# openclimatefix/predict_pv_yield

Measured on AMD Instinct MI355X. Metric: PV-site samples/sec (train step), conv3d 12->6 frames, higher is better.
Workload: dtype bf16; 1 GPU; conv3d train step (fwd + NMAE + bwd + Adam): sat [B,11,18,64,64] N(0,1), 4x Conv3d(3x3x3, 32ch) + fc 128/128/64, 128.6 M params; per_gpu_batch=32, global_batch=32, t_frames=18, parallelism=single

## Files before the change

predict_pv_yield_amd/csrc/linear_bf16.hip:

```cpp
#include "adam.h"
#include <string.h>

namespace pv {

template <int MT>
__global__ __launch_bounds__(256) void linear_fwd_bf16_kernel(const uint16_t* __restrict__ x,
                                                               const uint16_t* __restrict__ w,
                                                               float* __restrict__ partial, int m, int n,
                                                               long long k, int kblocks_per_wg) {
  const int lane = threadIdx.x & 63;
  const int wave = threadIdx.x >> 6;
  const int r = lane & 31, hh = lane >> 5;
  const int nt = blockIdx.y * 4 + wave;
  const long long total_kb = (k + 63) / 64;
  const long long kb0 = (long long)blockIdx.x * kblocks_per_wg;
  long long kb1 = kb0 + kblocks_per_wg;
  if (kb1 > total_kb) kb1 = total_kb;

  int wrow = nt * 32 + r;
  if (wrow > n - 1) wrow = n - 1;
  const uint16_t* wp = w + (size_t)wrow * k + 32 * hh;
  const uint16_t* xp[MT];
#pragma unroll
  for (int mt = 0; mt < MT; ++mt) {
// ... 450 lines not shown
#pragma unroll
    for (int q = 0; q < 4; ++q) {
      const uint16_t h0 = f32_to_bf16_bits(gx[2 * q]), h1 = f32_to_bf16_bits(gx[2 * q + 1]);
      const uint16_t l0 = f32_to_bf16_bits(gx[2 * q] - bf16_bits_to_f32(h0)), l1 = f32_to_bf16_bits(gx[2 * q + 1] - bf16_bits_to_f32(h1));
      hw[q] = (uint32_t)h0 | ((uint32_t)h1 << 16);
      lw[q] = (uint32_t)l0 | ((uint32_t)l1 << 16);
    }
    const bf16x8 bw = *reinterpret_cast<const bf16x8*>(wt + (32 * wave + col) * FD_WLD + 16 * st + 8 * half);
    o = __builtin_amdgcn_mfma_f32_32x32x16_bf16(__builtin_bit_cast(bf16x8, lw), bw, o, 0, 0, 0);
    o = __builtin_amdgcn_mfma_f32_32x32x16_bf16(__builtin_bit_cast(bf16x8, hw), bw, o, 0, 0, 0);
  }
  __syncthreads();
#pragma unroll
  for (int r = 0; r < 16; ++r) {
    const int b = (r & 3) + 8 * (r >> 2) + 4 * half;
    xs[b * FD_XLD + 32 * wave + col] = f32_to_bf16_bits(o[r]);
  }
  __syncthreads();
  for (int i = tid; i < 32 * (FD_KT / 8); i += 256) {
    const int b = i / (FD_KT / 8), c = i - b * (FD_KT / 8);
    if (b < m && k0 + 8 * c < k) {
      u32x4 o = *reinterpret_cast<const u32x4*>(xs + b * FD_XLD + 8 * c);
      if (gate_dx) {
        const u32x4 xv = *reinterpret_cast<const u32x4*>(x + (size_t)b * k + k0 + 8 * c);
#pragma unroll
        for (int q = 0; q < 4; ++q)
          o[q] &= __builtin_bit_cast(uint32_t, __builtin_bit_cast(u16x2_t, relu_pair01(xv[q])) * (u16x2_t){0xffff, 0xffff});
      }
      *reinterpret_cast<u32x4*>(dx + (size_t)b * k + k0 + 8 * c) = o;
    }
  }
}

constexpr int TL_XS = 320;
constexpr int TL_TS = 64 + 4;
constexpr int TL_GA = 2 * 4 * 3 * 64, TL_GD = 2 * 8 * 64;
typedef __attribute__((address_space(3))) s16x4 tl_lds_s16x4_t;
static_assert(32 * TL_XS <= FD_KT * FD_WLD * 2 && 4 * 32 * TL_TS * 4 <= FD_KT * FD_WLD * 2, "x block / transpose patches live in the weight tile's bytes");

__global__ __launch_bounds__(256) void tall_split_g_kernel(const float* __restrict__ dy, int m, int n, u32x4* __restrict__ ga,
                                                            u32x4* __restrict__ gd, int nblk) {
  const int total = nblk * (TL_GA + TL_GD);
  for (int f = blockIdx.x * blockDim.x + threadIdx.x; f < total; f += gridDim.x * blockDim.x) {
    const int mb = f / (TL_GA + TL_GD), i = f - mb * (TL_GA + TL_GD);
    float v[8];
    int term;
    if (i < TL_GA) {
      const int lane = i & 63, q = i >> 6, ks = q / 12, wave = (q / 3) & 3, r = lane & 31, hh = lane >> 5;
      term = q % 3;
#pragma unroll
      for (int j = 0; j < 8; ++j) {
        const int b = 32 * mb + 16 * ks + 8 * hh + j, nn = 32 * wave + r;
        v[j] = (b < m && nn < n) ? dy[(size_t)b * n + nn] : 0.f;
      }
    } else {
      const int i2 = i - TL_GA, lane = i2 & 63, q = i2 >> 6, st = q & 7, col = lane & 31, half = lane >> 5;
      term = q >> 3;
      const int b = 32 * mb + col;
#pragma unroll
      for (int j = 0; j < 8; ++j) {
        const int nn = 16 * st + 8 * half + j;
        v[j] = (b < m && nn < n) ? dy[(size_t)b * n + nn] : 0.f;
      }
    }
    u32x4 o;
#pragma unroll
// ... 565 lines not shown
    if (wave * 32 < n) {
#pragma unroll
      for (int ks = 0; ks < V3_KC / 16; ++ks) {
        const bf16x8 b = *reinterpret_cast<const bf16x8*>(tile + b_row + pos[ks]);
#pragma unroll
        for (int q = 0; q < MB; ++q) {
          const bf16x8 a = *reinterpret_cast<const bf16x8*>(tile + a_row + q * (32 * 256) + pos[ks]);
          acc[q] = __builtin_amdgcn_mfma_f32_32x32x16_bf16(a, b, acc[q], 0, 0, 0);
        }
      }
    }
  }
  const int col = wave * 32 + r;
  if (col < n) {
    float* dst = partial + (size_t)blockIdx.x * m * n + col;
#pragma unroll
    for (int q = 0; q < MB; ++q)
#pragma unroll
      for (int j = 0; j < 16; ++j) {
        const int row = 32 * q + (j & 3) + 8 * (j >> 2) + 4 * hh;
        if (row < m) dst[(size_t)row * n] = acc[q][j];
      }
  }
}

static int v3_split(long long k, int* tiles_per_wg, int* n_tiles) {
  const long long nt = (k + V3_KC - 1) / V3_KC;
  long long nwg = nt < 256 ? nt : 256;
  const long long per = (nt + nwg - 1) / nwg;
  nwg = (nt + per - 1) / per;
  *tiles_per_wg = (int)per;
  *n_tiles = (int)nt;
  return (int)nwg;
}

static bool v2_shapes(int m, int n) { return m <= 32 && n <= 128 && n % 16 == 0 && n >= 32; }
static int v2_split(long long k, int* tiles_per_wg, int* n_tiles) {
  const long long nt = (k + V2_KC - 1) / V2_KC;
  long long nwg = nt < 512 ? nt : 512;
  const long long per = (nt + nwg - 1) / nwg;
  nwg = (nt + per - 1) / per;
  *tiles_per_wg = (int)per;
  *n_tiles = (int)nt;
  return (int)nwg;
}

static int bf16_fwd_split(long long k, int* kblocks_per_wg) {
  long long total_kb = (k + 63) / 64;
  long long nwg = total_kb < 1024 ? total_kb : 1024;
  long long per = (total_kb + nwg - 1) / nwg;
  nwg = (total_kb + per - 1) / per;
  *kblocks_per_wg = (int)per;
  return (int)nwg;
}

}

using namespace pv;

extern "C" {

int pv_linear_bf16_workspace_bytes(int32_t m, int32_t n, int64_t k, size_t* bytes) {
  PV_REQUIRE(bytes && m > 0 && n > 0 && k > 0, PV_EINVAL, "pv_linear_bf16_workspace_bytes: bad arguments");
  int per;
  int nwg = bf16_fwd_split(k, &per);
  const size_t rows = (size_t)((m + 127) / 128) * 128;
// ... 112 lines not shown
  PV_REQUIRE(step >= 1, PV_EINVAL, "pv_linear_wgrad_adam_bf16: step must be >= 1");
  size_t lds = (size_t)m * BT * sizeof(float);
  PV_REQUIRE(lds <= 64 * 1024, PV_ESIZE, "pv_linear_wgrad_adam_bf16: m=%d too large", m);
  const AdamScalars ad = adam_scalars(lr, beta1, beta2, eps, step);
  unsigned kb = (unsigned)((k / 8 + 255) / 256);
  hipLaunchKernelGGL(linear_bwd_dw_bf16_kernel<1>, dim3(xcd_grid(kb, (unsigned)((n + BT - 1) / BT))), dim3(256), lds,
                     as_stream(stream), x, dy, y_relu_mask, param, m, n, (long long)k, exp_avg, exp_avg_sq, bf16_shadow, ad);
  return check_launch("pv_linear_wgrad_adam_bf16");
}

int pv_linear_wgrad_adam_f32(const float* x, const float* dy, const float* y_relu_mask, float* param, float* exp_avg,
                             float* exp_avg_sq, int32_t m, int32_t n, int64_t k, double lr, double beta1, double beta2,
                             double eps, int32_t step, void* stream) {
  PV_REQUIRE(x && dy && param && exp_avg && exp_avg_sq, PV_EINVAL, "pv_linear_wgrad_adam_f32: null pointer");
  PV_REQUIRE(m > 0 && n > 0 && k > 0 && k % 8 == 0, PV_ESIZE, "pv_linear_wgrad_adam_f32: bad sizes (k must be a multiple of 8)");
  PV_REQUIRE(((uintptr_t)x % 16) == 0 && ((uintptr_t)param % 16) == 0 && ((uintptr_t)exp_avg % 16) == 0 && ((uintptr_t)exp_avg_sq % 16) == 0,
             PV_EINVAL, "pv_linear_wgrad_adam_f32: 16-byte aligned buffers expected");
  PV_REQUIRE(step >= 1, PV_EINVAL, "pv_linear_wgrad_adam_f32: step must be >= 1");
  size_t lds = (size_t)m * BT * sizeof(float);
  PV_REQUIRE(lds <= 64 * 1024, PV_ESIZE, "pv_linear_wgrad_adam_f32: m=%d too large", m);
  const AdamScalars ad = adam_scalars(lr, beta1, beta2, eps, step);
  unsigned kb = (unsigned)((k / 8 + 255) / 256);
  hipLaunchKernelGGL((linear_bwd_dw_bf16_kernel<1, float>), dim3(xcd_grid(kb, (unsigned)((n + BT - 1) / BT))), dim3(256), lds,
                     as_stream(stream), x, dy, y_relu_mask, param, m, n, (long long)k, exp_avg, exp_avg_sq, (uint16_t*)nullptr, ad);
  return check_launch("pv_linear_wgrad_adam_f32");
}

#define PV_LAUNCH_FC1_ONE_PASS(grid, st, ...)                                                                         \
  do {                                                                                                                \
    const char* fs_ = getenv("PV_FC1_FETCH");                                                                         \
    if (fs_ && !strcmp(fs_, "late")) hipLaunchKernelGGL((linear_bwd_dw_dx_adam_kernel<1, false>), dim3(grid), dim3(256), 0, st, __VA_ARGS__); \
    else if (fs_ && !strcmp(fs_, "early1")) hipLaunchKernelGGL((linear_bwd_dw_dx_adam_kernel<1, true>), dim3(grid), dim3(256), 0, st, __VA_ARGS__); \
    else if (fs_ && !strcmp(fs_, "early2")) hipLaunchKernelGGL((linear_bwd_dw_dx_adam_kernel<2, true>), dim3(grid), dim3(256), 0, st, __VA_ARGS__); \
    else hipLaunchKernelGGL((linear_bwd_dw_dx_adam_kernel<2, true, 4>), dim3(grid), dim3(256), 0, st, __VA_ARGS__);    \
  } while (0)

int pv_linear_wgrad_dx_adam_bf16(const uint16_t* x, const float* dy, const float* y_relu_mask, float* param, float* exp_avg,
                                 float* exp_avg_sq, uint16_t* bf16_shadow, uint16_t* dx, float* db, int32_t m, int32_t n,
                                 int64_t k, double lr, double beta1, double beta2, double eps, int32_t step,
                                 int32_t gate_dx_by_x, int32_t moments_tiled, void* stream) {
  PV_REQUIRE(x && dy && param && exp_avg && exp_avg_sq, PV_EINVAL, "pv_linear_wgrad_dx_adam_bf16: null pointer");
  PV_REQUIRE(m > 0 && m <= 32 && n > 0 && n <= 128 && n % 8 == 0, PV_ESIZE,
             "pv_linear_wgrad_dx_adam_bf16: built for m <= 32 rows of x and n <= 128 (multiple of 8) outputs, got m=%d n=%d", m, n);
  PV_REQUIRE(k > 0 && k % 8 == 0, PV_ESIZE, "pv_linear_wgrad_dx_adam_bf16: k must be a multiple of 8");
  PV_REQUIRE(step >= 1, PV_EINVAL, "pv_linear_wgrad_dx_adam_bf16: step must be >= 1");
  PV_REQUIRE(!moments_tiled || k % FD_KT == 0, PV_ESIZE, "pv_linear_wgrad_dx_adam_bf16: tiled moments need k %% %d == 0", FD_KT);
  const AdamScalars ad = adam_scalars(lr, beta1, beta2, eps, step);
  const unsigned grid = (unsigned)((k + FD_KT - 1) / FD_KT);
  PV_LAUNCH_FC1_ONE_PASS(grid, as_stream(stream), x, dy, y_relu_mask, param, m, n,
                     (long long)k, exp_avg, exp_avg_sq, bf16_shadow, dx, db, ad, gate_dx_by_x, (const float*)nullptr,
                     moments_tiled ? 1 : 0);
  return check_launch("pv_linear_wgrad_dx_adam_bf16");
}

int pv_linear_wgrad_dx_adam_tall_bf16_workspace_bytes(int32_t m, size_t* bytes) {
  PV_REQUIRE(m > 0 && bytes, PV_EINVAL, "pv_linear_wgrad_dx_adam_tall_bf16_workspace_bytes: bad arguments");
  *bytes = (size_t)((m + 31) / 32) * (TL_GA + TL_GD) * 16;
  return PV_OK;
}

int pv_linear_wgrad_dx_adam_tall_bf16(const uint16_t* x, const float* dy, float* param, float* exp_avg, float* exp_avg_sq,
                                      uint16_t* bf16_shadow, uint16_t* dx, int32_t m, int32_t n, int64_t k, double lr,
                                      double beta1, double beta2, double eps, int32_t step, float grad_scale,
                                      int32_t gate_dx_by_x, int32_t moments_tiled, void* workspace, size_t workspace_bytes,
                                      void* stream) {
  PV_REQUIRE(x && dy && param && exp_avg && exp_avg_sq && workspace, PV_EINVAL, "pv_linear_wgrad_dx_adam_tall_bf16: null pointer");
  PV_REQUIRE(!moments_tiled || k % FD_KT == 0, PV_ESIZE, "pv_linear_wgrad_dx_adam_tall_bf16: tiled moments need k %% 128 == 0");
// ... 59 lines not shown
```

predict_pv_yield_amd/csrc/conv3d_wgrad_bf16_v2.hip:

```cpp
#include "pv_common.h"

namespace pv {

constexpr int W2TR = 8, W2TRI = 10, W2TW = 32, W2XW = 34;
constexpr int W2_SLAB_ELEMS = 28 * 32 * 32;
constexpr uint32_t W2_INVALID = 0x40000000u;

typedef __attribute__((address_space(3))) s16x4 w2_lds_s16x4;
typedef __attribute__((address_space(3))) unsigned char* w2_lds_ptr;
typedef int w2_i32x4 __attribute__((ext_vector_type(4)));

__device__ __forceinline__ void w2_lds_dma16(uint32_t lds_addr, uint32_t voff, w2_i32x4 rsrc, uint32_t soff) {
  asm volatile("s_mov_b32 m0, %0\n\ts_nop 0\n\tbuffer_load_dwordx4 %1, %2, %3 offen lds" ::"s"(lds_addr), "v"(voff), "s"(rsrc),
               "s"(soff)
               : "memory");
}
__device__ __forceinline__ w2_i32x4 w2_rsrc(const void* base, int bytes) {
  const uintptr_t a = (uintptr_t)base;
  return (w2_i32x4){(int)(uint32_t)a, (int)((a >> 32) & 0xffffu), bytes, 0x00020000};
}

#ifdef PV_DIAG_STAMPS
__device__ unsigned long long wgrad2_diag[PV_DIAG_WAVES * PV_DIAG_SLOTS];
#endif

template <int NACC, int Q>
__device__ __forceinline__ void w2_interleave() {
  if constexpr (Q < NACC) {
    constexpr int R = 2 + 2 * NACC;
    __builtin_amdgcn_sched_group_barrier(0x008, 1, 0);
    __builtin_amdgcn_sched_group_barrier(0x100, R / NACC + (Q < R % NACC ? 1 : 0), 0);
    w2_interleave<NACC, Q + 1>();
  }
}

template <int CPAD, bool F16 = false, bool PACK12 = false>
__global__ __launch_bounds__(512, 2) void conv3d_wgrad_bf16_v2_kernel(
    const uint16_t* __restrict__ x, const uint16_t* __restrict__ dy, float* __restrict__ slabs, int t_in, int h_in, int w_in,
    int t_out, int h_out, int w_out, int pad_t, int pad_h, int pad_w, int n_colblk, int t_chunk, int rpb) {
  constexpr int NCH = CPAD / 8;
  constexpr int VPR = 16 / NCH;
  constexpr int VOXB = CPAD * 2;
  constexpr int ROWB = W2XW * VOXB;
  constexpr int SLOTB = W2TRI * ROWB;
  constexpr int XVPP = 1024 / VOXB;
  constexpr int XPIECES = (W2XW + XVPP - 1) / XVPP;
  constexpr int XTAIL_LANES = (W2XW - (XPIECES - 1) * XVPP) * NCH;
  constexpr int DROWB = W2TW * 64;
  constexpr int DSLOTB = W2TR * DROWB;
  constexpr int NXS = 5;
  __shared__ __attribute__((aligned(1024))) unsigned char lds[NXS * SLOTB + 256 + 2 * DSLOTB];
  unsigned char* lds_const = lds + NXS * SLOTB;
  unsigned char* lds_dy = lds_const + 256;

  const int tid = threadIdx.x;
  const int lane = tid & 63;
  const int wave8 = __builtin_amdgcn_readfirstlane(tid >> 6);
  const bool loader = wave8 >= 4;
  const int wave = wave8 & 3;
  const int grp = lane >> 4;
  const int qi = (lane & 15) >> 2;
  const int pi = lane & 3;
  const int hh = grp >> 1;
  const int cb = 16 * (grp & 1);

  const int h0 = blockIdx.x * rpb;
  const int b = blockIdx.z;
  const int tc0 = blockIdx.y * t_chunk;
  const int tc1 = min(tc0 + t_chunk, t_out);
  const int wg_id = (blockIdx.z * gridDim.y + blockIdx.y) * gridDim.x + blockIdx.x;
  float* slab = slabs + (size_t)wg_id * W2_SLAB_ELEMS;

  static_assert(!PACK12 || CPAD == 16, "PACK12 packs the 16-channel image");
  constexpr bool PAIRED = CPAD == 16;
  constexpr int NACC = PACK12 ? 3 : (PAIRED ? 4 : 7);
  f32x16 acc[NACC];
#pragma unroll
  for (int i = 0; i < NACC; ++i)
#pragma unroll
    for (int j = 0; j < 16; ++j) acc[i][j] = 0.f;

  const int nt = tc1 - tc0, tn = nt + 2;
  const int n_items = nt > 0 ? nt * n_colblk : 0;
  const int u_end = tn * n_colblk;
  const uint32_t lds_base = __builtin_amdgcn_readfirstlane((uint32_t)(uintptr_t)(w2_lds_ptr)lds);

  if (n_items > 0 && loader) {
    const uint32_t x_plane_b = (uint32_t)h_in * w_in * CPAD * 2u, x_row_b = (uint32_t)w_in * CPAD * 2u;
    const uint32_t d_plane_b = (uint32_t)h_out * w_out * 64u, d_row_b = (uint32_t)w_out * 64u;
    const size_t x_sample = (size_t)t_in * h_in * w_in * CPAD, d_sample = (size_t)t_out * h_out * w_out * 32;
    const void* const x_base = x + (size_t)b * x_sample;
    const void* const d_base = dy + (size_t)b * d_sample;
    const int x_bytes = (int)(x_sample * 2), d_bytes = (int)(d_sample * 2);
    uint32_t xrow_src[3];
    bool xrow_in[3];
#pragma unroll
    for (int i = 0; i < 3; ++i) {
      const int hi = h0 - pad_h + wave + 4 * i;
      xrow_in[i] = (unsigned)hi < (unsigned)h_in && wave + 4 * i < rpb + 2;
      xrow_src[i] = xrow_in[i] ? (uint32_t)hi * x_row_b : 0u;
    }
    uint32_t drow_src[2];
    bool drow_in[2];
#pragma unroll
    for (int i = 0; i < 2; ++i) {
      const int ho = h0 + wave + 4 * i;
// ... 45 lines not shown
    for (int j = 0; j < n_items; ++j) {
      const int cb = j / nt, u0 = cb * tn + (j - cb * nt);
      __builtin_amdgcn_s_waitcnt(0x0f70);
      __syncthreads();
      if (next_u < u0 + 3) {
        for (; next_u < u0 + 3; ++next_u) x_slice(next_u);
        __builtin_amdgcn_s_waitcnt(0x0f70);
        __syncthreads();
      }
      for (; next_u <= u0 + 4 && next_u < u_end; ++next_u) x_slice(next_u);
      if (j + 1 < n_items) d_slice(j + 1);
    }
  } else if (n_items > 0) {
    if (tid < 64) reinterpret_cast<uint32_t*>(lds_const)[tid] = tid < 32 ? (F16 ? 0x3c003c00u : 0x3f803f80u) : 0u;

    int aoff[2];
#pragma unroll
    for (int s = 0; s < 2; ++s) {
      const int v = 8 * hh + 4 * s + qi;
      const int chunk = (cb + 4 * pi) >> 3;
      aoff[s] = v * 64 + ((chunk ^ ((v >> 2) & 3)) << 4) + (pi & 1) * 8;
    }
    int boff[NACC][2];
    int bkt[NACC];
    int my_tap[NACC];
#pragma unroll
    for (int i = 0; i < NACC; ++i) {
      int tap, c4 = 0;
      if constexpr (PACK12) {
        const int piece = 8 * (wave + 4 * i) + 4 * (grp & 1) + pi;
        tap = piece / 3;
        c4 = piece - 3 * tap;
        if (piece > 81) tap = 28;
      } else {
        tap = PAIRED ? 2 * (wave + 4 * i) + (grp & 1) : wave + 4 * i;
      }
      my_tap[i] = tap;
      if (tap > 26) tap = 26;
      const int kt = tap / 9, kh = (tap / 3) % 3, kw = tap % 3;
      bkt[i] = kt;
      const int cbx = PAIRED ? 0 : cb;
#pragma unroll
      for (int s = 0; s < 2; ++s) {
        const int v = kw + 8 * hh + 4 * s + qi;
        const int chunk = PACK12 ? (c4 >> 1) : ((cbx + 4 * pi) >> 3);
        const int sub = PACK12 ? (c4 & 1) : (pi & 1);
        boff[i][s] = kh * ROWB + v * VOXB + ((chunk ^ ((v / VPR) % NCH)) << 4) + sub * 8;
      }
    }
    typedef __attribute__((ext_vector_type(8))) short s16x8;
    const int last_tap = (PAIRED || PACK12) ? my_tap[NACC - 1] : (wave == 3 ? 27 : 0);
    const unsigned char* const_frag = last_tap < 27 ? nullptr : lds_const + (last_tap == 27 ? 0 : 128) + (lane & 15) * 8;

#ifdef PV_DIAG_STAMPS
    unsigned long long dg[PV_DIAG_SLOTS] = {0, 0, 0, 0, 0, 0, 0, 0}, s0, s1, s2;
#endif
    for (int j = 0; j < n_items; ++j) {
      const int cbj = j / nt, u0 = cbj * tn + (j - cbj * nt);
      PV_STAMP(s0);
      __syncthreads();
      if (cbj > 0 && j == cbj * nt) __syncthreads();
      PV_STAMP(s1);
      int slot_of_kt[3];
#pragma unroll
      for (int kt = 0; kt < 3; ++kt) slot_of_kt[kt] = ((u0 + kt) % NXS) * SLOTB;
      const unsigned char* dy_slot = lds_dy + (j & 1) * DSLOTB;
      int bslot[NACC];
#pragma unroll
      for (int i = 0; i < NACC; ++i) bslot[i] = bkt[i] == 0 ? slot_of_kt[0] : (bkt[i] == 1 ? slot_of_kt[1] : slot_of_kt[2]);
      auto read_step = [&](int st, s16x4 (&ra)[2], s16x4 (&rb)[NACC][2]) {
        const int rho = st >> 1, cg = st & 1;
        const unsigned char* ap = dy_slot + rho * DROWB + cg * 16 * 64;
        ra[0] = __builtin_amdgcn_ds_read_tr16_b64_v4i16((w2_lds_s16x4*)(ap + aoff[0]));
        ra[1] = __builtin_amdgcn_ds_read_tr16_b64_v4i16((w2_lds_s16x4*)(ap + aoff[1]));
        const int xo = rho * ROWB + cg * 16 * VOXB;
#pragma unroll
        for (int i = 0; i < NACC; ++i) {
          const unsigned char* bp = lds + bslot[i] + xo;
          const unsigned char* p0 = bp + boff[i][0];
          const unsigned char* p1 = bp + boff[i][1];
          if (i == NACC - 1) {
            p0 = const_frag ? const_frag : p0;
            p1 = const_frag ? const_frag : p1;
          }
          rb[i][0] = __builtin_amdgcn_ds_read_tr16_b64_v4i16((w2_lds_s16x4*)p0);
          rb[i][1] = __builtin_amdgcn_ds_read_tr16_b64_v4i16((w2_lds_s16x4*)p1);
        }
      };
      auto mfma_step = [&](const s16x4 (&ra)[2], const s16x4 (&rb)[NACC][2]) {
        const s16x8 a8 = {ra[0][0], ra[0][1], ra[0][2], ra[0][3], ra[1][0], ra[1][1], ra[1][2], ra[1][3]};
        typedef _Float16 w2_f16x8 __attribute__((ext_vector_type(8)));
#pragma unroll
        for (int i = 0; i < NACC; ++i) {
          s16x8 t8 = {rb[i][0][0], rb[i][0][1], rb[i][0][2], rb[i][0][3], rb[i][1][0], rb[i][1][1], rb[i][1][2], rb[i][1][3]};
          if constexpr (F16)
            acc[i] = __builtin_amdgcn_mfma_f32_32x32x16_f16(__builtin_bit_cast(w2_f16x8, a8), __builtin_bit_cast(w2_f16x8, t8), acc[i], 0, 0, 0);
          else
            acc[i] = __builtin_amdgcn_mfma_f32_32x32x16_bf16(__builtin_bit_cast(bf16x8, a8), __builtin_bit_cast(bf16x8, t8), acc[i], 0, 0, 0);
        }
      };
      s16x4 ra0[2], ra1[2], rb0[NACC][2], rb1[NACC][2];
      const bool skip_last_row = rpb < W2TR;
      read_step(0, ra0, rb0);
#pragma unroll
      for (int st = 0; st < W2TR * 2; st += 2) {
        if (st == W2TR * 2 - 2 && skip_last_row) break;
        __builtin_amdgcn_sched_barrier(0);
        read_step(st + 1, ra1, rb1);
        mfma_step(ra0, rb0);
        w2_interleave<NACC, 0>();
        __builtin_amdgcn_sched_barrier(0);
        if (st + 2 < W2TR * 2) {
          read_step(st + 2, ra0, rb0);
          mfma_step(ra1, rb1);
          w2_interleave<NACC, 0>();
        } else {
          mfma_step(ra1, rb1);
        }
        __builtin_amdgcn_sched_barrier(0);
      }
#ifdef PV_DIAG_STAMPS
      PV_STAMP(s2);
      dg[0] += s1 - s0;
      dg[1] += s2 - s1;
      dg[2] += 1;
#endif
    }
#ifdef PV_DIAG_STAMPS
    if (lane == 0 && wg_id * 4 + wave < PV_DIAG_WAVES)
      for (int i = 0; i < PV_DIAG_SLOTS; ++i) wgrad2_diag[(size_t)(wg_id * 4 + wave) * PV_DIAG_SLOTS + i] = dg[i];
#endif
  }
  if (loader) return;

  const int half = lane >> 5;
#pragma unroll
  for (int i = 0; i < NACC; ++i) {
    int tapslot = PAIRED ? 2 * (wave + 4 * i) + ((lane & 31) >> 4) : wave + 4 * i;
    int ci = PAIRED ? (lane & 15) : (lane & 31);
    if constexpr (PACK12) {
      const int piece = 8 * (wave + 4 * i) + ((lane & 31) >> 2);
      tapslot = piece / 3;
      ci = 4 * (piece - 3 * tapslot) + (lane & 3);
      if (piece > 81) tapslot = 28;
    }
    if (tapslot <= 27) {
      float* dst = slab + (size_t)tapslot * 1024 + ci;
#pragma unroll
      for (int j = 0; j < 16; ++j) {
        const int co = (j & 3) + 8 * (j >> 2) + 4 * half;
        dst[co * 32] = acc[i][j];
      }
    }
  }
}

void wgrad_v2_grid(const pv_conv3d_dims* d, int* n_rowblk, int* n_colblk, int* n_tchunk, int* t_chunk, int* rows_per_blk) {
  const int to = d->t_in + 2 * d->pad_t - 2, ho = d->h_in + 2 * d->pad_h - 2, wo = d->w_in + 2 * d->pad_w - 2;
  *n_rowblk = (ho + W2TR - 1) / W2TR;
  if ((long long)d->batch * *n_rowblk < 256 && (long long)d->batch * (*n_rowblk + 1) <= 256 &&
      (ho + *n_rowblk) / (*n_rowblk + 1) < (ho + *n_rowblk - 1) / *n_rowblk)
    *n_rowblk += 1;
  *rows_per_blk = (ho + *n_rowblk - 1) / *n_rowblk;
  *n_colblk = (wo + W2TW - 1) / W2TW;
  const long long tiles = (long long)d->batch * *n_rowblk;
  int max_chunks = (to + 1) / 2;
  if (max_chunks < 1) max_chunks = 1;
  int ntc = 1;
  long long best = -1;
  for (int c = 1; c <= max_chunks && tiles * c <= 16 * 256; ++c) {
    const int tch = (to + c - 1) / c, nch = (to + tch - 1) / tch;
    const long long rounds = (tiles * nch + 255) / 256;
    const long long cost = rounds * (tch + 2);
    if (best < 0 || cost < best) best = cost, ntc = nch;
  }
  *t_chunk = (to + ntc - 1) / ntc;
  *n_tchunk = (to + *t_chunk - 1) / *t_chunk;
}

size_t wgrad_v2_workspace_bytes(const pv_conv3d_dims* d) {
  int nrb, ncb, ntc, tch, rpb;
  wgrad_v2_grid(d, &nrb, &ncb, &ntc, &tch, &rpb);
  return (size_t)d->batch * nrb * ntc * W2_SLAB_ELEMS * sizeof(float);
}

int launch_conv3d_wgrad_bf16_v2(const uint16_t* x, const uint16_t* dy, float* slabs, const pv_conv3d_dims* d, int to, int ho,
                                int wo, hipStream_t st, int* n_slabs, bool f16) {
  if (((uintptr_t)x % 16) != 0 || ((uintptr_t)dy % 16) != 0) return 1;
  int nrb, ncb, ntc, tch, rpb;
  wgrad_v2_grid(d, &nrb, &ncb, &ntc, &tch, &rpb);
  *n_slabs = d->batch * nrb * ntc;
  dim3 grid((unsigned)nrb, (unsigned)ntc, (unsigned)d->batch);
#define PV_W2(CP, HALF)                                                                                                       \
  hipLaunchKernelGGL((conv3d_wgrad_bf16_v2_kernel<CP, HALF>), grid, dim3(512), 0, st, x, dy, slabs, d->t_in, d->h_in, d->w_in, to, \
                     ho, wo, d->pad_t, d->pad_h, d->pad_w, ncb, tch, rpb)
#define PV_W2P(HALF)                                                                                                        \
  hipLaunchKernelGGL((conv3d_wgrad_bf16_v2_kernel<16, HALF, true>), grid, dim3(512), 0, st, x, dy, slabs, d->t_in, d->h_in, d->w_in, \
                     to, ho, wo, d->pad_t, d->pad_h, d->pad_w, ncb, tch, rpb)
  if (pv_bf16_cpad(d->c_in) == 16) {
    const bool pack12 = d->c_in <= 12 && !getenv("PV_WGRAD_NO_PACK12");
    if (pack12) { if (f16) PV_W2P(true); else PV_W2P(false); }
    else { if (f16) PV_W2(16, true); else PV_W2(16, false); }
  } else { if (f16) PV_W2(32, true); else PV_W2(32, false); }
#undef PV_W2P
#undef PV_W2
  return 0;
}


constexpr int WR_GROUPS = 16;
__global__ __launch_bounds__(64 * WR_GROUPS) void conv3d_wgrad_reduce_kernel(const float* __restrict__ slabs, int n_slabs,
                                                                              float* __restrict__ dw, float* __restrict__ dbias,
                                                                              int c_out, int c_in) {
  __shared__ float part[WR_GROUPS][64];
  const int lane = threadIdx.x & 63, grp = threadIdx.x >> 6;
  const int i = blockIdx.x * 64 + lane;
  float s0 = 0.f, s1 = 0.f, s2 = 0.f, s3 = 0.f;
  for (int k = grp; k < n_slabs; k += 16 * WR_GROUPS) {
    float v[16];
#pragma unroll
    for (int j = 0; j < 16; ++j) v[j] = (k + WR_GROUPS * j < n_slabs) ? slabs[(size_t)(k + WR_GROUPS * j) * W2_SLAB_ELEMS + i] : 0.f;
#pragma unroll
    for (int j = 0; j < 16; j += 4) s0 += v[j], s1 += v[j + 1], s2 += v[j + 2], s3 += v[j + 3];
  }
  part[grp][lane] = (s0 + s1) + (s2 + s3);
  __syncthreads();
  if (grp == 0) {
    float t[WR_GROUPS];
#pragma unroll
    for (int q = 0; q < WR_GROUPS; ++q) t[q] = part[q][lane];
#pragma unroll
    for (int w = WR_GROUPS / 2; w >= 1; w >>= 1)
#pragma unroll
      for (int q = 0; q < w; ++q) t[q] = t[2 * q] + t[2 * q + 1];
    const float s = t[0];
    const int tap = i >> 10, co = (i >> 5) & 31, ci = i & 31;
// ... 103 lines not shown
```

Baseline: 20650 samples/s.

## Add warp-specialized persistent FC1 backward+Adam kernel with LDS DMA ring

Adds a new specialization of the fused fc1 weight-gradient, dx and Adam kernel. It dedicates four loader waves to streaming param, exp_avg, exp_avg_sq and x tiles into a four-stage LDS ring via buffer_load...lds DMA, while eight compute waves form gradients, apply Adam and compute dx. The grid is capped at the CU count so blocks are persistent and loop over tiles. The aim is to hide the memory latency of the bandwidth-bound optimizer update for the large fc1 weight. In exchange it relies on inline asm, a barrier hand-off between loader and compute waves that must stay matched, 32-bit buffer offsets, and an environment variable fallback to the old kernel.

```diff
diff --git a/predict_pv_yield_amd/csrc/linear_bf16.hip b/predict_pv_yield_amd/csrc/linear_bf16.hip
--- a/predict_pv_yield_amd/csrc/linear_bf16.hip
+++ b/predict_pv_yield_amd/csrc/linear_bf16.hip
@@ -506,6 +506,265 @@
   }
 }
 
+constexpr int FS_CHUNKB = 3 * 16 * 512;
+constexpr int FS_LW = 4;
+constexpr int FS_CL = 24 / FS_LW;
+constexpr int FS_XL = 8 / FS_LW;
+constexpr uint32_t FS_INVALID = 0xfffffff0u;
+typedef int fs_i32x4 __attribute__((ext_vector_type(4)));
+
+__device__ __forceinline__ void fs_lds_dma16(uint32_t lds_addr, uint32_t voff, fs_i32x4 rsrc) {
+  asm volatile("s_mov_b32 m0, %0\n\ts_nop 0\n\tbuffer_load_dwordx4 %1, %2, 0 offen lds" ::"s"(lds_addr), "v"(voff), "s"(rsrc)
+               : "memory");
+}
+__device__ __forceinline__ fs_i32x4 fs_rsrc(const void* base, uint32_t bytes) {
+  const uintptr_t a = (uintptr_t)base;
+  return (fs_i32x4){(int)(uint32_t)a, (int)((a >> 32) & 0xffffu), (int)bytes, 0x00020000};
+}
+
+template <int AHEAD, bool EARLY, int GR, int STAGES, int CW>
+__global__ __launch_bounds__(64 * (CW + FS_LW), 1) void linear_bwd_dw_dx_adam_kernel(
+    const uint16_t* __restrict__ x, const float* __restrict__ dy, const float* __restrict__ ymask, float* __restrict__ w,
+    int m, int n, long long k, float* __restrict__ exp_avg, float* __restrict__ exp_avg_sq, uint16_t* __restrict__ shadow,
+    uint16_t* __restrict__ dx, float* __restrict__ db, AdamScalars ad, int gate_dx, const float* __restrict__ ad_dev,
+    int mv_tiled) {
+  static_assert(GR == 4 && STAGES == 4 && (CW == 4 || CW == 8), "the ring's hand-over below is written for four stages and gradient halves");
+  constexpr int CPT = 32 / CW;
+  constexpr int KQN = FD_KT / CPT;
+  constexpr int NT = 64 * CW;
+  __shared__ __attribute__((aligned(1024))) unsigned char ring[STAGES * FS_CHUNKB];
+  __shared__ __attribute__((aligned(16))) float gs[32 * 128];
+  __shared__ __attribute__((aligned(16))) uint16_t wt[FD_KT * FD_WLD];
+  __shared__ __attribute__((aligned(1024))) uint16_t xt[32 * FD_KT];
+  typedef __attribute__((address_space(3))) unsigned char* fs_lds_ptr;
+  const int tid = threadIdx.x, lane = tid & 63;
+  const int wave = __builtin_amdgcn_readfirstlane(tid >> 6);
+  const int n_tiles = (int)(k / FD_KT);
+  const int n_my = (n_tiles - (int)blockIdx.x + (int)gridDim.x - 1) / (int)gridDim.x;
+  const int n_steps = 8 * n_my;
+
+  if (wave >= CW) {
+    const int lw = wave - CW;
+    const uint32_t ring_base = __builtin_amdgcn_readfirstlane((uint32_t)(uintptr_t)(fs_lds_ptr)ring);
+    const uint32_t xt_base = __builtin_amdgcn_readfirstlane((uint32_t)(uintptr_t)(fs_lds_ptr)xt);
+    const uint32_t w_bytes = (uint32_t)((size_t)n * k * 4);
+    const fs_i32x4 prs = fs_rsrc(w, w_bytes), mrs = fs_rsrc(exp_avg, w_bytes), vrs = fs_rsrc(exp_avg_sq, w_bytes);
+    const fs_i32x4 xrs = fs_rsrc(x, (uint32_t)((size_t)m * k * 2));
+    const int slot = lane >> 5, pos = lane & 31;
+    const uint32_t piece_b = (uint32_t)(CW == 4 ? 2 * (pos & 15) + (pos >> 4) : pos) * 16u;
+    const uint32_t row_b = (uint32_t)k * 4u;
+    auto request = [&](int s) __attribute__((always_inline)) {
+      const int i = s & 7;
+      const uint32_t t = blockIdx.x + (uint32_t)(s >> 3) * gridDim.x;
+      if (i == 0) {
+        const uint32_t col_b = t * (uint32_t)(FD_KT * 2);
+#pragma unroll
+        for (int q = 0; q < FS_XL; ++q) {
+          const int b = 4 * (lw + FS_LW * q) + (lane >> 4);
+          const uint32_t off = b < m ? (uint32_t)b * ((uint32_t)k * 2u) + col_b + (uint32_t)(lane & 15) * 16u : FS_INVALID;
+          fs_lds_dma16(xt_base + (uint32_t)(lw + FS_LW * q) * 1024u, off, xrs);
+        }
+      }
+      const uint32_t dst = ring_base + (uint32_t)(s & (STAGES - 1)) * FS_CHUNKB;
+      const uint32_t p_col_b = t * (uint32_t)(FD_KT * 4);
+      const uint32_t mv_tile_b = t * (uint32_t)n * (uint32_t)(FD_KT * 4);
+#pragma unroll
+      for (int a = 0; a < 3; ++a)
+#pragma unroll
+        for (int q = 0; q < FS_CL / 3; ++q) {
+          const int pr = lw + FS_LW * q;
+          const int row = 8 * (2 * pr + slot) + i;
+          uint32_t off = FS_INVALID;
+          if (row < n) {
+            if (a == 0 || !mv_tiled) off = (uint32_t)row * row_b + p_col_b + piece_b;
+            else off = mv_tile_b + (uint32_t)row * (uint32_t)(FD_KT * 4) + piece_b;
+          }
+          fs_lds_dma16(dst + (uint32_t)(a * 8192) + (uint32_t)pr * 1024u, off, a == 0 ? prs : a == 1 ? mrs : vrs);
+        }
+    };
+    for (int s = 0; s < STAGES - 1 && s < n_steps; ++s) request(s);
+    for (int s = 0; s < n_steps; ++s) {
+      if (s + 2 < n_steps) asm volatile("s_waitcnt vmcnt(%0)" ::"n"(2 * FS_CL) : "memory");
+      else asm volatile("s_waitcnt vmcnt(0)" ::: "memory");
+      __syncthreads();
+      if (s + STAGES - 1 < n_steps) request(s + STAGES - 1);
+      if ((s & 7) == 7 && dx) {
+        __syncthreads();
+        __syncthreads();
+        __syncthreads();
+      }
+    }
+    return;
+  }
+
+  if (ad_dev) ad = adam_scalars_load(ad_dev);
+  const int kq = tid & (KQN - 1), rg = tid / KQN;
+  for (int i = tid; i < 32 * 128; i += NT) {
+    const int b = i >> 7, nn = i & 127;
+    float v = 0.f;
+    if (b < m && nn < n) {
+      const size_t off = (size_t)b * n + nn;
+      v = dy[off];
+      if (ymask && !(ymask[off] > 0.f)) v = 0.f;
+    }
+    gs[i] = v;
+  }
+  typedef float f32x2_t __attribute__((ext_vector_type(2)));
+  typedef uint32_t u32x2_t __attribute__((ext_vector_type(2)));
+  f32x2_t acc2[GR][CPT / 2];
+  auto form_gradient = [&](int r0) __attribute__((always_inline)) {
+#pragma unroll
+    for (int i = 0; i < GR; ++i)
+#pragma unroll
+      for (int j = 0; j < CPT / 2; ++j) acc2[i][j] = (f32x2_t){0.f, 0.f};
+#pragma unroll 4
+    for (int b = 0; b < m; ++b) {
+      uint32_t raw[CPT / 2];
+      if constexpr (CPT == 8) {
+        const u32x4 r4 = *reinterpret_cast<const u32x4*>(xt + b * FD_KT + CPT * kq);
+        raw[0] = r4[0], raw[1] = r4[1], raw[CPT / 2 - 2] = r4[2], raw[CPT / 2 - 1] = r4[3];
+      } else {
+        const u32x2_t r2 = *reinterpret_cast<const u32x2_t*>(xt + b * FD_KT + CPT * kq);
+        raw[0] = r2[0], raw[1] = r2[1];
+      }
+      f32x2_t xv2[CPT / 2];
+#pragma unroll
+      for (int q = 0; q < CPT / 2; ++q)
+        xv2[q] = (f32x2_t){__builtin_bit_cast(float, raw[q] << 16), __builtin_bit_cast(float, raw[q] & 0xffff0000u)};
+      const f32x4 g0 = *reinterpret_cast<const f32x4*>(gs + b * 128 + 8 * rg + (r0 & 4));
+#pragma unroll
+      for (int i = 0; i < GR; ++i) {
+        const float gv = g0[(r0 & 3) + i];
+        const f32x2_t g2 = {gv, gv};
+#pragma unroll
+        for (int j = 0; j < CPT / 2; ++j) acc2[i][j] = __builtin_elementwise_fma(g2, xv2[j], acc2[i][j]);
+      }
+    }
+  };
+  const int col = lane & 31, half = lane >> 5;
+  for (int jt = 0; jt < n_my; ++jt) {
+    const long long k0 = ((long long)blockIdx.x + (long long)jt * gridDim.x) * FD_KT;
+    const long long kc = k0 + CPT * kq;
+    const size_t mv_tile_base = (size_t)(k0 / FD_KT) * (size_t)n * FD_KT + CPT * kq;
+    uint32_t wold[8][CPT / 2];
+    u32x4 xg[512 / NT];
+#pragma unroll
+    for (int i = 0; i < 8; ++i) {
+      __syncthreads();
+      if (i == 0 && jt == 0 && db && blockIdx.x == 0 && tid < n) {
+        float sacc = 0.f;
+        for (int b = 0; b < m; ++b) sacc += gs[b * 128 + tid];
+        db[tid] = sacc;
+      }
+      if (i % GR == 0) form_gradient(i);
+      if (i == 4) {
+#pragma unroll
+        for (int it = 0; it < 512 / NT; ++it) xg[it] = *reinterpret_cast<const u32x4*>(xt + 8 * (tid + NT * it));
+      }
+      const unsigned char* rowp = ring + (i & (STAGES - 1)) * FS_CHUNKB + rg * 512 + kq * 16;
+      float pv[CPT], mv[CPT], vv[CPT];
+#pragma unroll
+      for (int h = 0; h < CPT / 4; ++h) {
+        *reinterpret_cast<f32x4*>(pv + 4 * h) = *reinterpret_cast<const f32x4*>(rowp + 256 * h);
+        *reinterpret_cast<f32x4*>(mv + 4 * h) = *reinterpret_cast<const f32x4*>(rowp + 8192 + 256 * h);
+        *reinterpret_cast<f32x4*>(vv + 4 * h) = *reinterpret_cast<const f32x4*>(rowp + 16384 + 256 * h);
+      }
+      const bool row_ok = 8 * rg + i < n;
+#pragma unroll
+      for (int q = 0; q < CPT / 2; ++q)
+        wold[i][q] = row_ok ? (pack_bf16_pair(pv[2 * q], pv[2 * q + 1])) : 0u;
+      if (row_ok) {
+        const size_t off = (size_t)(8 * rg + i) * k + kc;
+        uint32_t sh[CPT / 2];
+#pragma unroll
+        for (int j = 0; j < CPT; ++j) {
+          adam_update(pv[j], mv[j], vv[j], acc2[i % GR][j >> 1][j & 1], ad);
+          const float pp = pv[j];
+          if (j & 1) sh[j >> 1] |= (uint32_t)f32_to_bf16_bits(pp) << 16; else sh[j >> 1] = f32_to_bf16_bits(pp);
+        }
+        const size_t moff = mv_tiled ? mv_tile_base + (size_t)(8 * rg + i) * FD_KT : off;
+#pragma unroll
+        for (int h = 0; h < CPT / 4; ++h) {
+          *reinterpret_cast<f32x4*>(w + off + 4 * h) = *reinterpret_cast<const f32x4*>(pv + 4 * h);
+          *reinterpret_cast<f32x4*>(exp_avg + moff + 4 * h) = *reinterpret_cast<const f32x4*>(mv + 4 * h);
+          *reinterpret_cast<f32x4*>(exp_avg_sq + moff + 4 * h) = *reinterpret_cast<const f32x4*>(vv + 4 * h);
+        }
+        if (shadow) {
+          if constexpr (CPT == 8) {
+            u32x4 so = {sh[0], sh[1], sh[CPT / 2 - 2], sh[CPT / 2 - 1]};
+            *reinterpret_cast<u32x4*>(shadow + off) = so;
+          } else {
+            const uint32_t n0 = (uint32_t)__builtin_amdgcn_mov_dpp((int)sh[0], 0xB1, 0xf, 0xf, true);
+            const uint32_t n1 = (uint32_t)__builtin_amdgcn_mov_dpp((int)sh[1], 0xB1, 0xf, 0xf, true);
+            if (!(kq & 1)) {
+              u32x4 so = {sh[0], sh[1], n0, n1};
+              *reinterpret_cast<u32x4*>(shadow + off) = so;
+            }
+          }
+        }
+      }
+    }
+    if (!dx) continue;
+#pragma unroll
+    for (int j = 0; j < CPT; ++j) {
+      u32x4 piece;
+#pragma unroll
+      for (int q = 0; q < 4; ++q) {
+        const uint32_t lo = (wold[2 * q][j >> 1] >> (16 * (j & 1))) & 0xffffu;
+        const uint32_t hi = (wold[2 * q + 1][j >> 1] >> (16 * (j & 1))) & 0xffffu;
+        piece[q] = lo | (hi << 16);
+      }
+      *reinterpret_cast<u32x4*>(wt + (CPT * kq + j) * FD_WLD + 8 * rg) = piece;
+    }
+    __syncthreads();
+    f32x16 o;
+    if (wave < 4) {
+#pragma unroll
+      for (int r = 0; r < 16; ++r) o[r] = 0.f;
+#pragma unroll
+      for (int st = 0; st < 8; ++st) {
+        const f32x4 a0 = *reinterpret_cast<const f32x4*>(gs + col * 128 + 16 * st + 8 * half);
+        const f32x4 a1 = *reinterpret_cast<const f32x4*>(gs + col * 128 + 16 * st + 8 * half + 4);
+        const float gx[8] = {a0[0], a0[1], a0[2], a0[3], a1[0], a1[1], a1[2], a1[3]};
+        u32x4 hw, lw;
+#pragma unroll
+        for (int q = 0; q < 4; ++q) {
+          const uint16_t h0 = f32_to_bf16_bits(gx[2 * q]), h1 = f32_to_bf16_bits(gx[2 * q + 1]);
+          const uint16_t l0 = f32_to_bf16_bits(gx[2 * q] - bf16_bits_to_f32(h0)), l1 = f32_to_bf16_bits(gx[2 * q + 1] - bf16_bits_to_f32(h1));
+          hw[q] = (uint32_t)h0 | ((uint32_t)h1 << 16);
+          lw[q] = (uint32_t)l0 | ((uint32_t)l1 << 16);
+        }
+        const bf16x8 bw = *reinterpret_cast<const bf16x8*>(wt + (32 * wave + col) * FD_WLD + 16 * st + 8 * half);
+        o = __builtin_amdgcn_mfma_f32_32x32x16_bf16(__builtin_bit_cast(bf16x8, lw), bw, o, 0, 0, 0);
+        o = __builtin_amdgcn_mfma_f32_32x32x16_bf16(__builtin_bit_cast(bf16x8, hw), bw, o, 0, 0, 0);
+      }
+    }
+    __syncthreads();
+    if (wave < 4) {
+#pragma unroll
+      for (int r = 0; r < 16; ++r) {
+        const int b = (r & 3) + 8 * (r >> 2) + 4 * half;
+        wt[b * FD_XLD + 32 * wave + col] = f32_to_bf16_bits(o[r]);
+      }
+    }
+    __syncthreads();
+#pragma unroll
+    for (int it = 0; it < 512 / NT; ++it) {
+      const int i = tid + NT * it;
+      const int b = i / (FD_KT / 8), c = i - b * (FD_KT / 8);
+      if (b < m) {
+        u32x4 ov = *reinterpret_cast<const u32x4*>(wt + b * FD_XLD + 8 * c);
+        if (gate_dx) {
+#pragma unroll
+          for (int q = 0; q < 4; ++q)
+            ov[q] &= __builtin_bit_cast(uint32_t, __builtin_bit_cast(u16x2_t, relu_pair01(xg[it][q])) * (u16x2_t){0xffff, 0xffff});
+        }
+        *reinterpret_cast<u32x4*>(dx + (size_t)b * k + k0 + 8 * c) = ov;
+      }
+    }
+  }
+}
+
 constexpr int TL_XS = 320;
 constexpr int TL_TS = 64 + 4;
 constexpr int TL_GA = 2 * 4 * 3 * 64, TL_GD = 2 * 8 * 64;
@@ -1137,6 +1396,17 @@
   *tiles_per_wg = (int)per;
   *n_tiles = (int)nt;
   return (int)nwg;
+}
+
+static bool fc1_stream_covers(int m, int n, long long k) {
+  return k % FD_KT == 0 && (unsigned long long)n * (unsigned long long)k * 4ull < 0xfffffff0ull &&
+         (unsigned long long)m * (unsigned long long)k * 2ull < 0xfffffff0ull;
+}
+static unsigned fc1_stream_grid(unsigned n_tiles) {
+  int dev = 0, cus = 0;
+  if (hipGetDevice(&dev) != hipSuccess || hipDeviceGetAttribute(&cus, hipDeviceAttributeMultiprocessorCount, dev) != hipSuccess || cus <= 0)
+    cus = 256;
+  return n_tiles < (unsigned)cus ? n_tiles : (unsigned)cus;
 }
 
 static bool v2_shapes(int m, int n) { return m <= 32 && n <= 128 && n % 16 == 0 && n >= 32; }
@@ -1315,7 +1585,9 @@
     if (fs_ && !strcmp(fs_, "late")) hipLaunchKernelGGL((linear_bwd_dw_dx_adam_kernel<1, false>), dim3(grid), dim3(256), 0, st, __VA_ARGS__); \
     else if (fs_ && !strcmp(fs_, "early1")) hipLaunchKernelGGL((linear_bwd_dw_dx_adam_kernel<1, true>), dim3(grid), dim3(256), 0, st, __VA_ARGS__); \
     else if (fs_ && !strcmp(fs_, "early2")) hipLaunchKernelGGL((linear_bwd_dw_dx_adam_kernel<2, true>), dim3(grid), dim3(256), 0, st, __VA_ARGS__); \
-    else hipLaunchKernelGGL((linear_bwd_dw_dx_adam_kernel<2, true, 4>), dim3(grid), dim3(256), 0, st, __VA_ARGS__);    \
+    else if ((fs_ && !strcmp(fs_, "early2h")) || !fc1_stream_covers(m, n, k))                                         \
+      hipLaunchKernelGGL((linear_bwd_dw_dx_adam_kernel<2, true, 4>), dim3(grid), dim3(256), 0, st, __VA_ARGS__);       \
+    else hipLaunchKernelGGL((linear_bwd_dw_dx_adam_kernel<2, true, 4, 4, 8>), dim3(fc1_stream_grid(grid)), dim3(768), 0, st, __VA_ARGS__); \
   } while (0)
 
 int pv_linear_wgrad_dx_adam_bf16(const uint16_t* x, const float* dy, const float* y_relu_mask, float* param, float* exp_avg,
```

Result: faster. 21010 samples/s, median of 6 (+1.7%).

## Add sliding-window tap assignment to reuse x rows across kh in 32-ch wgrad

Applied to the files above, without the earlier changes.

For the 32-channel weight-gradient kernel, each wave is now assigned taps that share the same kt/kw and differ only in kh. This lets it keep a rolling 3-row register window of x fragments and load one new row per step instead of re-reading a separate x fragment for every tap. The goal is to cut LDS transposed reads per MFMA, since the inner loop is bound by LDS reads. The cost is more VGPRs held for the window and a different interleave ratio, which could pressure occupancy at 2 blocks per CU. It is enabled by default and can be disabled with an environment variable.

```diff
diff --git a/predict_pv_yield_amd/csrc/conv3d_wgrad_bf16_v2.hip b/predict_pv_yield_amd/csrc/conv3d_wgrad_bf16_v2.hip
--- a/predict_pv_yield_amd/csrc/conv3d_wgrad_bf16_v2.hip
+++ b/predict_pv_yield_amd/csrc/conv3d_wgrad_bf16_v2.hip
@@ -24,17 +24,22 @@
 __device__ unsigned long long wgrad2_diag[PV_DIAG_WAVES * PV_DIAG_SLOTS];
 #endif
 
-template <int NACC, int Q>
+template <int NACC, int R, int Q>
 __device__ __forceinline__ void w2_interleave() {
   if constexpr (Q < NACC) {
-    constexpr int R = 2 + 2 * NACC;
     __builtin_amdgcn_sched_group_barrier(0x008, 1, 0);
     __builtin_amdgcn_sched_group_barrier(0x100, R / NACC + (Q < R % NACC ? 1 : 0), 0);
-    w2_interleave<NACC, Q + 1>();
-  }
-}
-
-template <int CPAD, bool F16 = false, bool PACK12 = false>
+    w2_interleave<NACC, R, Q + 1>();
+  }
+}
+
+__device__ __forceinline__ int w2_slide_tap(int wave, int i) {
+  if (i == 6) return wave < 3 ? 20 + 3 * wave : 27;
+  const int g = 2 * wave + i / 3, kt = g / 3;
+  return 9 * kt + 3 * (i % 3) + (g - 3 * kt);
+}
+
+template <int CPAD, bool F16 = false, bool PACK12 = false, bool SLIDE = false>
 __global__ __launch_bounds__(512, 2) void conv3d_wgrad_bf16_v2_kernel(
     const uint16_t* __restrict__ x, const uint16_t* __restrict__ dy, float* __restrict__ slabs, int t_in, int h_in, int w_in,
     int t_out, int h_out, int w_out, int pad_t, int pad_h, int pad_w, int n_colblk, int t_chunk, int rpb) {
@@ -72,6 +77,7 @@
   float* slab = slabs + (size_t)wg_id * W2_SLAB_ELEMS;
 
   static_assert(!PACK12 || CPAD == 16, "PACK12 packs the 16-channel image");
+  static_assert(!SLIDE || CPAD == 32, "the sliding window is the 32-channel form");
   constexpr bool PAIRED = CPAD == 16;
   constexpr int NACC = PACK12 ? 3 : (PAIRED ? 4 : 7);
   f32x16 acc[NACC];
@@ -183,6 +189,8 @@
         tap = piece / 3;
         c4 = piece - 3 * tap;
         if (piece > 81) tap = 28;
+      } else if constexpr (SLIDE) {
+        tap = w2_slide_tap(wave, i);
       } else {
         tap = PAIRED ? 2 * (wave + 4 * i) + (grp & 1) : wave + 4 * i;
       }
@@ -200,7 +208,7 @@
       }
     }
     typedef __attribute__((ext_vector_type(8))) short s16x8;
-    const int last_tap = (PAIRED || PACK12) ? my_tap[NACC - 1] : (wave == 3 ? 27 : 0);
+    const int last_tap = (PAIRED || PACK12 || SLIDE) ? my_tap[NACC - 1] : (wave == 3 ? 27 : 0);
     const unsigned char* const_frag = last_tap < 27 ? nullptr : lds_const + (last_tap == 27 ? 0 : 128) + (lane & 15) * 8;
 
 #ifdef PV_DIAG_STAMPS
@@ -219,56 +227,120 @@
       int bslot[NACC];
 #pragma unroll
       for (int i = 0; i < NACC; ++i) bslot[i] = bkt[i] == 0 ? slot_of_kt[0] : (bkt[i] == 1 ? slot_of_kt[1] : slot_of_kt[2]);
-      auto read_step = [&](int st, s16x4 (&ra)[2], s16x4 (&rb)[NACC][2]) {
-        const int rho = st >> 1, cg = st & 1;
-        const unsigned char* ap = dy_slot + rho * DROWB + cg * 16 * 64;
-        ra[0] = __builtin_amdgcn_ds_read_tr16_b64_v4i16((w2_lds_s16x4*)(ap + aoff[0]));
-        ra[1] = __builtin_amdgcn_ds_read_tr16_b64_v4i16((w2_lds_s16x4*)(ap + aoff[1]));
-        const int xo = rho * ROWB + cg * 16 * VOXB;
-#pragma unroll
-        for (int i = 0; i < NACC; ++i) {
-          const unsigned char* bp = lds + bslot[i] + xo;
-          const unsigned char* p0 = bp + boff[i][0];
-          const unsigned char* p1 = bp + boff[i][1];
-          if (i == NACC - 1) {
-            p0 = const_frag ? const_frag : p0;
-            p1 = const_frag ? const_frag : p1;
+      const bool skip_last_row = rpb < W2TR;
+      typedef _Float16 w2_f16x8 __attribute__((ext_vector_type(8)));
+      auto mfma1 = [&](f32x16& c, const s16x8 a8, const s16x4 b0, const s16x4 b1) {
+        const s16x8 t8 = {b0[0], b0[1], b0[2], b0[3], b1[0], b1[1], b1[2], b1[3]};
+        if constexpr (F16)
+          c = __builtin_amdgcn_mfma_f32_32x32x16_f16(__builtin_bit_cast(w2_f16x8, a8), __builtin_bit_cast(w2_f16x8, t8), c, 0, 0, 0);
+        else
+          c = __builtin_amdgcn_mfma_f32_32x32x16_bf16(__builtin_bit_cast(bf16x8, a8), __builtin_bit_cast(bf16x8, t8), c, 0, 0, 0);
+      };
+      if constexpr (SLIDE) {
+        const unsigned char* gp[2][2];
+        const unsigned char* lp[2];
+#pragma unroll
+        for (int s = 0; s < 2; ++s) {
+          gp[0][s] = lds + bslot[0] + boff[0][s];
+          gp[1][s] = lds + bslot[3] + boff[3][s];
+          lp[s] = lds + bslot[6] + boff[6][s];
+        }
+        s16x4 win[2][3][2][2], ra[2][2], rl[2][2];
+        auto read_row = [&](int r, int cg) {
+#pragma unroll
+          for (int gi = 0; gi < 2; ++gi)
+#pragma unroll
+            for (int s = 0; s < 2; ++s)
+              win[gi][r % 3][cg][s] = __builtin_amdgcn_ds_read_tr16_b64_v4i16((w2_lds_s16x4*)(gp[gi][s] + r * ROWB + cg * 16 * VOXB));
+        };
+        auto read_step = [&](int st) {
+          const int rho = st >> 1, cg = st & 1;
+          const unsigned char* ap = dy_slot + rho * DROWB + cg * 16 * 64;
+          ra[st & 1][0] = __builtin_amdgcn_ds_read_tr16_b64_v4i16((w2_lds_s16x4*)(ap + aoff[0]));
+          ra[st & 1][1] = __builtin_amdgcn_ds_read_tr16_b64_v4i16((w2_lds_s16x4*)(ap + aoff[1]));
+          read_row(rho + 2, cg);
+#pragma unroll
+          for (int s = 0; s < 2; ++s) {
+            const unsigned char* p = lp[s] + rho * ROWB + cg * 16 * VOXB;
+            rl[st & 1][s] = __builtin_amdgcn_ds_read_tr16_b64_v4i16((w2_lds_s16x4*)(const_frag ? const_frag : p));
           }
-          rb[i][0] = __builtin_amdgcn_ds_read_tr16_b64_v4i16((w2_lds_s16x4*)p0);
-          rb[i][1] = __builtin_amdgcn_ds_read_tr16_b64_v4i16((w2_lds_s16x4*)p1);
+        };
+        auto mfma_step = [&](int st) {
+          const int rho = st >> 1, cg = st & 1, par = st & 1;
+          const s16x8 a8 = {ra[par][0][0], ra[par][0][1], ra[par][0][2], ra[par][0][3],
+                            ra[par][1][0], ra[par][1][1], ra[par][1][2], ra[par][1][3]};
+#pragma unroll
+          for (int gi = 0; gi < 2; ++gi)
+#pragma unroll
+            for (int kh = 0; kh < 3; ++kh) mfma1(acc[3 * gi + kh], a8, win[gi][(rho + kh) % 3][cg][0], win[gi][(rho + kh) % 3][cg][1]);
+          mfma1(acc[6], a8, rl[par][0], rl[par][1]);
+        };
+        read_row(0, 0);
+        read_row(0, 1);
+        read_row(1, 0);
+        read_row(1, 1);
+        read_step(0);
+#pragma unroll
+        for (int st = 0; st < W2TR * 2; st += 2) {
+          if (st == W2TR * 2 - 2 && skip_last_row) break;
+          __builtin_amdgcn_sched_barrier(0);
+          read_step(st + 1);
+          mfma_step(st);
+          w2_interleave<NACC, 8, 0>();
+          __builtin_amdgcn_sched_barrier(0);
+          if (st + 2 < W2TR * 2) {
+            read_step(st + 2);
+            mfma_step(st + 1);
+            w2_interleave<NACC, 8, 0>();
+          } else {
+            mfma_step(st + 1);
+          }
+          __builtin_amdgcn_sched_barrier(0);
         }
-      };
-      auto mfma_step = [&](const s16x4 (&ra)[2], const s16x4 (&rb)[NACC][2]) {
-        const s16x8 a8 = {ra[0][0], ra[0][1], ra[0][2], ra[0][3], ra[1][0], ra[1][1], ra[1][2], ra[1][3]};
-        typedef _Float16 w2_f16x8 __attribute__((ext_vector_type(8)));
-#pragma unroll
-        for (int i = 0; i < NACC; ++i) {
-          s16x8 t8 = {rb[i][0][0], rb[i][0][1], rb[i][0][2], rb[i][0][3], rb[i][1][0], rb[i][1][1], rb[i][1][2], rb[i][1][3]};
-          if constexpr (F16)
-            acc[i] = __builtin_amdgcn_mfma_f32_32x32x16_f16(__builtin_bit_cast(w2_f16x8, a8), __builtin_bit_cast(w2_f16x8, t8), acc[i], 0, 0, 0);
-          else
-            acc[i] = __builtin_amdgcn_mfma_f32_32x32x16_bf16(__builtin_bit_cast(bf16x8, a8), __builtin_bit_cast(bf16x8, t8), acc[i], 0, 0, 0);
+      } else {
+        auto read_step = [&](int st, s16x4 (&ra)[2], s16x4 (&rb)[NACC][2]) {
+          const int rho = st >> 1, cg = st & 1;
+          const unsigned char* ap = dy_slot + rho * DROWB + cg * 16 * 64;
+          ra[0] = __builtin_amdgcn_ds_read_tr16_b64_v4i16((w2_lds_s16x4*)(ap + aoff[0]));
+          ra[1] = __builtin_amdgcn_ds_read_tr16_b64_v4i16((w2_lds_s16x4*)(ap + aoff[1]));
+          const int xo = rho * ROWB + cg * 16 * VOXB;
+#pragma unroll
+          for (int i = 0; i < NACC; ++i) {
+            const unsigned char* bp = lds + bslot[i] + xo;
+            const unsigned char* p0 = bp + boff[i][0];
+            const unsigned char* p1 = bp + boff[i][1];
+            if (i == NACC - 1) {
+              p0 = const_frag ? const_frag : p0;
+              p1 = const_frag ? const_frag : p1;
+            }
+            rb[i][0] = __builtin_amdgcn_ds_read_tr16_b64_v4i16((w2_lds_s16x4*)p0);
+            rb[i][1] = __builtin_amdgcn_ds_read_tr16_b64_v4i16((w2_lds_s16x4*)p1);
+          }
+        };
+        auto mfma_step = [&](const s16x4 (&ra)[2], const s16x4 (&rb)[NACC][2]) {
+          const s16x8 a8 = {ra[0][0], ra[0][1], ra[0][2], ra[0][3], ra[1][0], ra[1][1], ra[1][2], ra[1][3]};
+#pragma unroll
+          for (int i = 0; i < NACC; ++i) mfma1(acc[i], a8, rb[i][0], rb[i][1]);
+        };
+        s16x4 ra0[2], ra1[2], rb0[NACC][2], rb1[NACC][2];
+        read_step(0, ra0, rb0);
+#pragma unroll
+        for (int st = 0; st < W2TR * 2; st += 2) {
+          if (st == W2TR * 2 - 2 && skip_last_row) break;
+          __builtin_amdgcn_sched_barrier(0);
+          read_step(st + 1, ra1, rb1);
+          mfma_step(ra0, rb0);
+          w2_interleave<NACC, 2 + 2 * NACC, 0>();
+          __builtin_amdgcn_sched_barrier(0);
+          if (st + 2 < W2TR * 2) {
+            read_step(st + 2, ra0, rb0);
+            mfma_step(ra1, rb1);
+            w2_interleave<NACC, 2 + 2 * NACC, 0>();
+          } else {
+            mfma_step(ra1, rb1);
+          }
+          __builtin_amdgcn_sched_barrier(0);
         }
-      };
-      s16x4 ra0[2], ra1[2], rb0[NACC][2], rb1[NACC][2];
-      const bool skip_last_row = rpb < W2TR;
-      read_step(0, ra0, rb0);
-#pragma unroll
-      for (int st = 0; st < W2TR * 2; st += 2) {
-        if (st == W2TR * 2 - 2 && skip_last_row) break;
-        __builtin_amdgcn_sched_barrier(0);
-        read_step(st + 1, ra1, rb1);
-        mfma_step(ra0, rb0);
-        w2_interleave<NACC, 0>();
-        __builtin_amdgcn_sched_barrier(0);
-        if (st + 2 < W2TR * 2) {
-          read_step(st + 2, ra0, rb0);
-          mfma_step(ra1, rb1);
-          w2_interleave<NACC, 0>();
-        } else {
-          mfma_step(ra1, rb1);
-        }
-        __builtin_amdgcn_sched_barrier(0);
       }
 #ifdef PV_DIAG_STAMPS
       PV_STAMP(s2);
@@ -287,7 +359,7 @@
   const int half = lane >> 5;
 #pragma unroll
   for (int i = 0; i < NACC; ++i) {
-    int tapslot = PAIRED ? 2 * (wave + 4 * i) + ((lane & 31) >> 4) : wave + 4 * i;
+    int tapslot = PAIRED ? 2 * (wave + 4 * i) + ((lane & 31) >> 4) : (SLIDE ? w2_slide_tap(wave, i) : wave + 4 * i);
     int ci = PAIRED ? (lane & 15) : (lane & 31);
     if constexpr (PACK12) {
       const int piece = 8 * (wave + 4 * i) + ((lane & 31) >> 2);
@@ -342,17 +414,21 @@
   wgrad_v2_grid(d, &nrb, &ncb, &ntc, &tch, &rpb);
   *n_slabs = d->batch * nrb * ntc;
   dim3 grid((unsigned)nrb, (unsigned)ntc, (unsigned)d->batch);
-#define PV_W2(CP, HALF)                                                                                                       \
-  hipLaunchKernelGGL((conv3d_wgrad_bf16_v2_kernel<CP, HALF>), grid, dim3(512), 0, st, x, dy, slabs, d->t_in, d->h_in, d->w_in, to, \
-                     ho, wo, d->pad_t, d->pad_h, d->pad_w, ncb, tch, rpb)
+#define PV_W2(CP, HALF, SL)                                                                                                  \
+  hipLaunchKernelGGL((conv3d_wgrad_bf16_v2_kernel<CP, HALF, false, SL>), grid, dim3(512), 0, st, x, dy, slabs, d->t_in, d->h_in, \
+                     d->w_in, to, ho, wo, d->pad_t, d->pad_h, d->pad_w, ncb, tch, rpb)
 #define PV_W2P(HALF)                                                                                                        \
   hipLaunchKernelGGL((conv3d_wgrad_bf16_v2_kernel<16, HALF, true>), grid, dim3(512), 0, st, x, dy, slabs, d->t_in, d->h_in, d->w_in, \
                      to, ho, wo, d->pad_t, d->pad_h, d->pad_w, ncb, tch, rpb)
   if (pv_bf16_cpad(d->c_in) == 16) {
     const bool pack12 = d->c_in <= 12 && !getenv("PV_WGRAD_NO_PACK12");
     if (pack12) { if (f16) PV_W2P(true); else PV_W2P(false); }
-    else { if (f16) PV_W2(16, true); else PV_W2(16, false); }
-  } else { if (f16) PV_W2(32, true); else PV_W2(32, false); }
+    else { if (f16) PV_W2(16, true, false); else PV_W2(16, false, false); }
+  } else if (!getenv("PV_WGRAD_NO_SLIDE")) {
+    if (f16) PV_W2(32, true, true); else PV_W2(32, false, true);
+  } else {
+    if (f16) PV_W2(32, true, false); else PV_W2(32, false, false);
+  }
 #undef PV_W2P
 #undef PV_W2
   return 0;
```

After: 21010 samples/s before, 20930 samples/s after. No clear change (-0.4%).
